# Fable3/CarND-Path-Planning-Project

Hardware: AMD Instinct MI355X
Metric: candidate trajectories/sec (spline+cost, 50-pt horizon) at 1/2/4/8 MI355X (higher is better)
Workload: dtype f64

## Files before the change

carnd-path-planning-project_amd/csrc/pp_api.h:

```cpp
#pragma once

extern "C" {

void pp_params_default(pp_params* p) {
    if (!p) return;
    memset(p, 0, sizeof(*p));
    p->n_points = 50;
    p->n_speeds = 5;
    p->cost_mode = PP_COST_REFERENCE;
    p->emit_paths = 0;
    const double offs[4] = {-4.0, -2.0, 0.0, 2.0};
    for (int i = 0; i < 4; i++) p->speed_offsets[i] = offs[i];
    p->relaxed_acc = 5;
    p->min_relaxed_acc_while_braking = 4;
    p->maximum_acc = 8;
    p->max_speed = 22.2;
    p->car_length = 4.5;
    p->safety_distance = 2;
    p->keep_distance = 10;
    p->keep_distance_leeway = 0.5;
    p->n_draws = 0;
    p->noise_seed = 0x5EED0002ull;
    p->noise_first_scene = 0;
    p->noise_pos_sigma = 0.5;
// ... 151 lines not shown
}

int32_t pp_map_geometry(const pp_map* M, double* out, int32_t n) {
    if (!M || !out || n != M->n) return PP_ERR_ARG;
    memcpy(out, M->ptab.data(), sizeof(double) * (4 + 2 * NL) * (size_t)n);
    return PP_OK;
}

int32_t pp_reserve(pp_map* M, int32_t device, int64_t max_scenes) {
    if (!M || device < 0 || device >= kMaxDev || max_scenes < 0) return PP_ERR_ARG;
    std::lock_guard<std::mutex> lk(M->mu);
    DeviceGuard g(device);
    int rc = dev_init(M, device);
    if (rc) return rc;
    StreamWS& W = M->dev[device].sws[nullptr];
    rc = ensure_ws(W, nullptr, max_scenes);
    return rc ? rc : ensure_rec(W, nullptr, max_scenes);
}

int32_t pp_eval(pp_map* M, const pp_scene_batch* in, const pp_params* prm, pp_result* out,
                int32_t device, void* hip_stream) {
    return eval_impl(M, in, prm, out, device, hip_stream, nullptr);
}

int32_t pp_debug_set(int32_t key, int32_t value) {
    bool ok = false;
    switch (key) {
        case PP_DBG_PREP_GROUP: ok = prep_group_ok(value); break;
        case PP_DBG_PREP_WAVES: ok = value == 0 || value == 3 || value == 4; break;
        case PP_DBG_SHAPE: ok = value >= 0 && value <= PP_SHAPE_STEP; break;
        case PP_DBG_POISON: ok = value == 0 || value == 1; break;
        case PP_DBG_SPLIT: ok = value >= 0 && value <= 2; break;
        case PP_DBG_SORT_CARS: ok = value >= 0 && value <= 2; break;
        default: break;
    }
    if (!ok) return PP_ERR_ARG;
    g_dbg[key].store(value, std::memory_order_relaxed);
    return PP_OK;
}

int32_t pp_debug_get(int32_t key) { return key >= 0 && key < PP_DBG_KEYS ? dbg(key) : PP_ERR_ARG; }

int32_t pp_timing_enable(pp_map* M, int32_t device, int32_t enable) {
    if (!M || device < 0 || device >= kMaxDev) return PP_ERR_ARG;
    std::lock_guard<std::mutex> lk(M->mu);
    DevState& D = M->dev[device];
    D.timing = enable == PP_TIMING_K2 ? 2 : (enable != 0 ? 1 : 0);
    if (D.timing) {
        DeviceGuard g(device);
        const int rc = dev_init(M, device);
        if (rc) return rc;
        while (D.ev.pool.size() + D.ev.rec.size() < 4 * kSplitMax * 256) {
            hipEvent_t e;
            if (hipEventCreate(&e) != hipSuccess) return PP_ERR_HIP;
            D.ev.pool.push_back(e);
        }
    }
    return PP_OK;
}

int32_t pp_timing_read(pp_map* M, int32_t device, double* ms3, int64_t* launches3) {
    if (!M || device < 0 || device >= kMaxDev || !ms3 || !launches3) return PP_ERR_ARG;
    std::lock_guard<std::mutex> lk(M->mu);
    DevState& D = M->dev[device];
    DeviceGuard g(device);
    for (int k = 0; k < 3; k++) { ms3[k] = 0; launches3[k] = 0; }
// ... 117 lines not shown
```

carnd-path-planning-project_amd/csrc/pp_host_map.h:

```cpp
#pragma once

namespace {

constexpr int kMaxDev = 16;
constexpr int kMaxWaypoints = 1 << 24;
constexpr int kPrepD = 12 + 4 * NL;
constexpr int kPrepI = 7;

template <class H, hipError_t (*kRelease)(H)>
class Owned {
    H h_ = nullptr;
public:
    Owned() = default;
    Owned(Owned&& o) noexcept { std::swap(h_, o.h_); }
    Owned& operator=(Owned&& o) noexcept { std::swap(h_, o.h_); return *this; }
    ~Owned() { reset(); }
    H get() const { return h_; }
    explicit operator bool() const { return h_ != nullptr; }
    void reset() { if (h_) (void)kRelease(h_); h_ = nullptr; }
    H* out() { reset(); return &h_; }
};
using Stream = Owned<hipStream_t, hipStreamDestroy>;
using Event = Owned<hipEvent_t, hipEventDestroy>;
struct Pinned : Owned<void*, hipHostFree> {
// ... 12 lines not shown
public:
    DevMem() = default;
    DevMem(DevMem&& o) noexcept { *this = std::move(o); }
    DevMem& operator=(DevMem&& o) noexcept { std::swap(p_, o.p_); std::swap(cap_, o.cap_); return *this; }
    ~DevMem() { reset(); }
    T* get() const { return p_; }
    int64_t cap() const { return cap_; }
    explicit operator bool() const { return p_ != nullptr; }
    void reset() { if (p_) (void)hipFree(p_); p_ = nullptr; cap_ = 0; }
    int grow(hipStream_t st, int64_t cap, size_t bytes) {
        if (cap_ >= cap) return PP_OK;
        if (p_) { (void)hipStreamSynchronize(st); reset(); }
        if (hipMalloc((void**)&p_, bytes) != hipSuccess) { p_ = nullptr; (void)hipGetLastError(); return PP_ERR_NOMEM; }
        cap_ = cap;
        return PP_OK;
    }
    int alloc(size_t n) { return grow(nullptr, (int64_t)n, sizeof(T) * n); }
};
struct EventSet {
    std::vector<hipEvent_t> pool;
    std::vector<hipEvent_t> rec;
    std::vector<int> kind;
    EventSet() = default;
    EventSet(EventSet&& o) noexcept { *this = std::move(o); }
    EventSet& operator=(EventSet&& o) noexcept { pool.swap(o.pool); rec.swap(o.rec); kind.swap(o.kind); return *this; }
    ~EventSet() {
        for (auto* v : {&pool, &rec})
            for (hipEvent_t e : *v) { Event own; *own.out() = e; }
    }
};

constexpr int kSplitMax = 4;
constexpr int kPartMax = 16;
struct StreamWS {
    DevMem<> ws;
    DevMem<> rec;
    DevMem<uint32_t> gbits;
    DevMem<> srt;
    Stream st2[kSplitMax - 1];
    Event fork, join[kSplitMax - 1];
};
struct DevTables {
    DevMem<double> map;
    DevMem<double> lanetab;
    DevMem<uint2> wgrid;
    DevMem<double2> wseg;
    DevMem<double> atab;
};
struct DevRes {
    bool init = false;
    DevTables tab;
    DevMem<double> arctab;
    std::map<void*, StreamWS> sws;
    DevMem<> frame;
    Pinned frame_host;
    Stream frame_stream;
    DevMem<> stage;
    Pinned stage_host;
    EventSet ev;
};
struct DevState : DevRes {
    uint32_t frame_seq = 0;
    std::mutex frame_mu;
    std::mutex stage_mu;
    pptab::CarTable plan_table;
    int timing = 0;
};

}

struct pp_map {
    int n = 0;
    std::vector<double> geom;
    std::vector<double> ptab;
    std::vector<double> lanetab;
    std::vector<double> arctab;
    int fastm = 0;
    std::vector<uint2> wgrid;
    std::vector<double2> wseg;
    std::vector<double> atab;
    WGrid wg;
    DevState dev[kMaxDev];
    std::mutex mu;
};

namespace {

struct DeviceGuard {
    int prev = -1;
    explicit DeviceGuard(int d) { if (hipGetDevice(&prev) != hipSuccess) prev = -1; (void)hipSetDevice(d); }
    ~DeviceGuard() { if (prev >= 0) (void)hipSetDevice(prev); }
};

void fill_arctab(pp_map* M) {
    M->arctab.assign(ppfollow::arc_doubles(M->n), 0.0);
    ppfollow::build_arc(M->lanetab.data() + 2 * NL * (size_t)M->n, M->n, M->arctab.data());
}

void fill_ptab(pp_map* M) {
// ... 284 lines not shown
```

carnd-path-planning-project_amd/csrc/pp_k_cand.h:

```cpp
#pragma once

struct CandRes { double acc_sum, travelled; int ng; uint32_t flags; uint64_t adj0, adj1; };

template <bool kLarge, int kOutMode>
__device__ CandRes run_candidate(const pp_params& P, const Slot& sl, double cx, double cy,
                                 double angle, double ca0, double sa0, SC sc, int room, double* wx,
                                 double* wy, int64_t ws, double* px, int64_t ps, bool out_on = true,
                                 double* rec = nullptr, int dcls = 0, int64_t rs = 0) {
    (void)dcls;
    const bool kOut = kOutMode == 2 || kOutMode == 4;
    const bool kRec = kOutMode == 3 && out_on;
    const int64_t rstride = (int64_t)room * ws;
    CandRes R;
    R.acc_sum = 0; R.travelled = 0; R.ng = 0; R.flags = 0; R.adj0 = 0; R.adj1 = 0;
    const int nk = sl.m(0), ncp = sl.m(1), npk = sl.m(2), mflags = sl.m(3);
    if (mflags & kMetaTrunc) R.flags |= PP_ST_SPLINE_TRUNC;
    if (mflags & kMetaWalkFail) R.flags |= PP_ST_NAN;
    double pos_x = 0, pos_y = 0;
    OutFrame F = {cx, cy, ca0, sa0};
    double opx = cx, opy = cy;
    (void)angle;
    double cur_t = 0.02;
    int ng = 0;
    if (mflags & kMetaFallback) {
// ... 358 lines not shown
    for (int i = K + ng; i < N; i++) {
        if (!PP_CHKP(out.next_x + (int64_t)i * S + s, nx, nnext, 10)) break;
        out.next_x[(int64_t)i * S + s] = 0; out.next_y[(int64_t)i * S + s] = 0;
    }
    out.n_out[s] = K + ng;
    out.winner[s] = c;
}

template <bool kSlow>
__device__ __forceinline__ void cand_status(const PrepV& pv, const pp_result& out, const CandSm& L, int64_t s0,
                                            int nsc, int D, int BPS, int tid) {
    if (tid < nsc && ((L.sSlow[tid] != 0) == kSlow) && PP_CHK(s0 + tid < g_lim.nscen, 15, s0 + tid)) {
        const uint32_t st = (uint32_t)pv.status[(s0 + tid) * D] | L.sFlags[tid];
        if (BPS == 1) out.status[s0 + tid] = st;
        else atomicOr(&out.status[s0 + tid], st);
    }
}

template <bool kSlow>
__device__ __forceinline__ void cand_store_slot(const CandSm& L, int nslot, double* wslot, int64_t s0, int nsc,
                                                int NS, int tid) {
    constexpr int kItems = 5 * kWinKnots + 4;
    for (int idx = tid; idx < nsc * kItems; idx += (int)blockDim.x) {
        const int w = idx / kItems, e = idx - w * kItems;
        if ((L.sSlow[w] != 0) != kSlow) continue;
        const int64_t s = s0 + w;
        const Slot sl = lds_slot(L.sX, nslot, L.sMeta, w * NL + L.sNg[w] / NS);
        double* rec_s = wslot + s * kWinRec;
        if (e < 5 * kWinKnots) rec_s[e] = sl.X[e];
        else ((int*)(rec_s + 5 * kWinKnots))[e - 5 * kWinKnots] = sl.m(e - 5 * kWinKnots);
    }
}

template <bool kSlow, int kMode, int kEmitIn = 0, bool kPreA = false>
__device__ __forceinline__ void cand_group(const MapG& mg, const pp_scene_batch& in, const pp_params& P,
                                           const PrepV& pv, const pp_result& out, int SPB, int BPS,
                                           double* rec, uint64_t* adjm, int64_t g, double* sm,
                                           double* wslot = nullptr) {
    constexpr bool emit_in = kEmitIn == 1 && kMode == 1;
    constexpr bool win_inline = kEmitIn == 2 && kMode == 1;
    const int NS = P.n_speeds, Cv = NL * NS, N = P.n_points;
    const int D = P.n_draws > 1 ? P.n_draws : 1;
    const int C = D * Cv;
    const int nslot = NL * SPB;
    double* sX = sm;
    double* sY = sX + nslot * kKP;
    double* sA = sY + nslot * kKP;
    double* sB = sA + nslot * kKP;
    double* sC = sB + nslot * kKP;
    int* sMeta = (int*)(sC + nslot * kKP);
    uint32_t* sFlags = (uint32_t*)(sMeta + 4 * nslot);
    const MapV m = map_view(mg.buf, mg.n);
    const int64_t S = in.n_scenes;
    const int64_t Sv = S * D;
    int64_t s0;
    int coff;
    int nsc;
    if (BPS == 1) { s0 = g * SPB; coff = 0; }
    else if (BPS < 0) { s0 = g * 256 / C; coff = (int)(g * 256 - s0 * C); }
    else { s0 = g / BPS; coff = (int)(g - s0 * BPS) * 256; }
    if (BPS < 0) {
        const int span = (coff + 255) / C + 1;
        nsc = (int)((S - s0) < span ? (S - s0) : span);
    } else {
        nsc = (int)((S - s0) < SPB ? (S - s0) : SPB);
    }
    const int tid = threadIdx.x;
    uint32_t* sSlow = sFlags + SPB;
    uint64_t* sAdj = (uint64_t*)(((uintptr_t)(sSlow + SPB) + 7) & ~(uintptr_t)7);
    int* sNg = (int*)(sAdj + 2 * SPB);
    double* sCost = (double*)(((uintptr_t)(sNg + SPB) + 7) & ~(uintptr_t)7);
    if (tid < SPB) { sFlags[tid] = 0; sSlow[tid] = 0; }
#ifdef PP_TRACE
    if (!kSlow && tid == 0) {
        PP_TRACE_AT(blockIdx.x, 0);
        if (blockIdx.x < (unsigned)kTraceK1) g_trace[8 * blockIdx.x + 7] = trace_hwid();
    }
#endif
#ifdef PP_CHECK
    if (!kPreA) {
        for (int i = tid; i < 5 * nslot * kKP; i += (int)blockDim.x) sX[i] = __builtin_nan("");
        for (int i = tid; i < 4 * nslot; i += (int)blockDim.x) sMeta[i] = kMetaPoison;
    }
#endif
    __syncthreads();
    bool mine = false;
    for (int t = tid; t < nsc * D; t += (int)blockDim.x) {
        const int q = t / D;
        if (pv.lim_mask[(s0 + q) * D + (t - q * D)] & kLimSlow) { atomicOr(&sSlow[q], 1u); mine = true; }
    }
    if (!__syncthreads_or(mine) && kSlow) return;
    if (!kPreA) {
        int TS = (int)blockDim.x / nslot;
        if (TS > 8) TS = 8;
        const int j = tid / TS, r = tid - j * TS;
        const bool act = j < NL * nsc && ((sSlow[j / NL] != 0) == kSlow);
        const Slot sl = lds_slot(sX, nslot, sMeta, j);
        const int L = j % NL;
        const int64_t s = s0 + j / NL;
        LaneGeom g;
        PP_REGION_A("a1");
        if (act) { g = lane_geom(pv, s * D, Sv, L); team_a1(m, in, g, s, L, sl, r, TS); }
        __syncthreads();
        PP_REGION_A("a2");
        const int js = tid;
        const bool act_s = js < NL * nsc && ((sSlow[js / NL] != 0) == kSlow);
        const Slot sls = lds_slot(sX, nslot, sMeta, js);
        if (act_s) {
            const int64_t vs = (s0 + js / NL) * D;
            LaneGeom gs;
            gs.K = pv.K[vs];
            gs.npk = gs.K > 0 ? gs.K - 1 : 0;
            gs.pos_x = pv.pos_x[vs]; gs.pos_y = pv.pos_y[vs]; gs.ego_d = pv.ego_d[vs];
            team_a2(gs, sls);
        }
        __syncthreads();
        PP_REGION_A("a3");
        if (act) team_a3(sl, r, TS);
        __syncthreads();
        PP_REGION_A("a4");
        if (act_s) team_a4(sls);
        __syncthreads();
        PP_REGION_A("a5");
        if (act) team_a5(sl, r, TS);
// ... 140 lines not shown
            double sr, cr;
            turn_sincos<true>(rt, sr, cr);
            pcr[idx] = cr; psr[idx] = sr;
        }
        __syncthreads();
        if (!kSlow && tid == 0) PP_TRACE_AT(blockIdx.x, 7);
        if (tid < nsc && ((sSlow[tid] != 0) == kSlow)) {
            const int64_t s = s0 + tid;
            emit_scene_pre<kEmitChunk>(in, P, pv, out, rec, s, pv.K[s], sNg[tid], sAdj[2 * tid],
                                          sAdj[2 * tid + 1], pcr + tid * N, psr + tid * N);
        }
    }
}

template <bool kSlow, int kMode>
__global__ __launch_bounds__(256) __attribute__((amdgpu_waves_per_eu(kCandWaves))) void k_cand(MapG mg, pp_scene_batch in, pp_params P, PrepV pv,
                                              pp_result out, int SPB, int BPS, double* rec, uint64_t* adjm,
                                              uint32_t* gbits, int64_t ngroups, const uint32_t* glist,
                                              const uint32_t* gcount, int64_t g0, double* wslot) {
    extern __shared__ __attribute__((aligned(16))) double sm[];
    if (!kSlow) {
        cand_group<false, kMode>(mg, in, P, pv, out, SPB, BPS, rec, adjm, g0 + blockIdx.x, sm, wslot);
        return;
    }
    const uint32_t nl = *gcount;
    for (uint32_t i = blockIdx.x; i < nl; i += gridDim.x) {
        const int64_t g = glist[i];
        if (!PP_CHK(g < ngroups, 21, g)) continue;
        __syncthreads();
        cand_group<true, kMode>(mg, in, P, pv, out, SPB, BPS, rec, adjm, g, sm, wslot);
        if (threadIdx.x == 0) atomicAnd(&gbits[g >> 5], ~(1u << (g & 31)));
    }
}
```

carnd-path-planning-project_amd/csrc/pp_k_spline.h:

```cpp
#pragma once

struct Slot {
    double *X, *Y, *A, *B, *C;
    int* meta;
    int64_t st;
    int64_t mst;
    __device__ __forceinline__ double& x(int i) const { return X[i * st]; }
    __device__ __forceinline__ double& y(int i) const { return Y[i * st]; }
    __device__ __forceinline__ double& a(int i) const { return A[i * st]; }
    __device__ __forceinline__ double& b(int i) const { return B[i * st]; }
    __device__ __forceinline__ double& c(int i) const { return C[i * st]; }
    __device__ __forceinline__ int& m(int k) const { return meta[k * mst]; }
};
__device__ __forceinline__ Slot lds_slot(double* sX, int nslot, int* sMeta, int j) {
    (void)nslot;
    double* b = sX + (int64_t)j * kKP * 5;
    return Slot{b, b + 1, b + 2, b + 3, b + 4, sMeta + 4 * j, 5, 1};
}
constexpr int kCandCostLanes = 256;
struct CandLds {
    int spb;
    static __host__ __device__ constexpr size_t up8(size_t b) { return (b + 7) / 8 * 8; }
    __host__ __device__ constexpr int nslot() const { return NL * spb; }
    __host__ __device__ constexpr int slot_doubles() const { return 5 * kKP * nslot(); }
    __host__ __device__ constexpr size_t meta() const { return sizeof(double) * 5 * kKP * nslot(); }
    __host__ __device__ constexpr size_t flags() const { return meta() + sizeof(int) * 4 * nslot(); }
    __host__ __device__ constexpr size_t slow() const { return flags() + sizeof(uint32_t) * spb; }
    __host__ __device__ constexpr size_t adj() const { return up8(slow() + sizeof(uint32_t) * spb); }
    __host__ __device__ constexpr size_t ng() const { return adj() + sizeof(uint64_t) * 2 * spb; }
    __host__ __device__ constexpr size_t bytes() const { return ng() + sizeof(int) * spb; }
    __host__ __device__ constexpr size_t cost() const { return up8(bytes()); }
    __host__ __device__ constexpr size_t bytes_cost() const { return cost() + sizeof(double) * kCandCostLanes; }
    __host__ __device__ constexpr int doubles() const {
        return (int)(((sizeof(double) * 5 * kKP * (NL * spb) + sizeof(int) * 4 * (NL * spb) + sizeof(uint32_t) * 2 * spb + 7) / 8 * 8 +
                      sizeof(uint64_t) * 2 * spb + sizeof(int) * spb + 7) / 8);
    }
    __host__ __device__ constexpr bool replay_fits(int N) const { return 2 * spb * N <= slot_doubles(); }
};
#if PP_NUM_LANES == 3
static_assert(CandLds{1}.bytes() == 2116 && CandLds{4}.bytes() == 8464 && CandLds{16}.bytes() == 33856, "k_cand's LDS");
static_assert(CandLds{1}.bytes_cost() == 4168 && CandLds{4}.bytes_cost() == 10512 &&
              CandLds{16}.bytes_cost() == 35904, "k_cand's LDS with the cost array");
#elif PP_NUM_LANES == 4
static_assert(CandLds{1}.bytes() == 2812 && CandLds{4}.bytes() == 11248 && CandLds{16}.bytes() == 44992, "k_cand's LDS");
static_assert(CandLds{1}.bytes_cost() == 4864 && CandLds{4}.bytes_cost() == 13296 &&
              CandLds{16}.bytes_cost() == 47040, "k_cand's LDS with the cost array");
#endif
static_assert(8u * CandLds{1}.doubles() >= CandLds{1}.bytes() && 8u * CandLds{4}.doubles() >= CandLds{4}.bytes() &&
              8u * CandLds{16}.doubles() >= CandLds{16}.bytes(), "doubles() covers bytes()");
static_assert(CandLds{1}.doubles() == (CandLds{1}.bytes() + 7) / 8 && CandLds{4}.doubles() == (CandLds{4}.bytes() + 7) / 8 &&
              CandLds{16}.doubles() == (CandLds{16}.bytes() + 7) / 8, "doubles() is bytes() rounded up");
constexpr int kMetaFallback = 1, kMetaTrunc = 2, kMetaWalkFail = 4;

__device__ void setup_lane(const MapV& m, const pp_params& P, const pp_scene_batch& in,
                           const PrepV& pv, int64_t s, int64_t v, int64_t Sv, int L, const Slot& sl) {
    const int64_t S = in.n_scenes;
    const int K = pv.K[v];
    const double pos_x = pv.pos_x[v], pos_y = pv.pos_y[v];
    const double ca = pv.ca_m[v], sa = pv.sa_m[v];
    const double start = pv.ego_speed[v], ego_d = pv.ego_d[v], ego_vd = pv.ego_vd[v];
    const int ref_wp = pv.ref_wp[v];
    const double ratio = pv.ratio[L * Sv + v];
    int flags = 0;
    double min_cpd = start * 1;
    min_cpd = s_max(min_cpd, 5.0);
    const double d_diff = lane_offset(L) - ego_d;
    const double d_acc = 4;
    bool slow = false;
    double lst = 2.0;
    if ((ego_vd < 0) == (d_diff < 0)) {
        const double dmax = ego_vd * ego_vd / d_acc / 2;
// ... 263 lines not shown
```

carnd-path-planning-project_amd/csrc/pp_launch.h:

```cpp
#pragma once

namespace {

size_t prep_bytes(int64_t S) { return ((size_t)S * (kPrepD * 8 + kPrepI * 4) + 255) / 256 * 256; }
size_t rec_bytes(int64_t S) { return (size_t)S * (3 * PP_MAX_POINTS + 2) * 8 + 256; }
static_assert(kWinRec <= 3 * PP_MAX_POINTS + 2, "the stored winner slots share the record's memory");
double* rec_buf(void* rec) { return (double*)rec; }
uint64_t* adj_buf(void* rec, int64_t cap) { return (uint64_t*)((double*)rec + 3 * PP_MAX_POINTS * cap); }

PrepV prep_bind(void* base, int64_t S) {
    PrepV p;
    double* d = (double*)base;
    double** dd[] = {&p.pos_x, &p.pos_y, &p.angle, &p.ca_m, &p.sa_m, &p.ca_p, &p.sa_p,
                     &p.ego_speed, &p.ego_d, &p.ego_vd, &p.in_ts, &p.in_tt};
    int k = 0;
    for (double** q : dd) *q = d + (int64_t)(k++) * S;
    p.ratio = d + (int64_t)(k) * S; k += NL;
    p.l_ts = d + (int64_t)(k) * S; k += NL;
    p.l_tt = d + (int64_t)(k) * S; k += NL;
    p.score = d + (int64_t)(k) * S; k += NL;
    int32_t* ip = (int32_t*)(d + (int64_t)kPrepD * S);
    int32_t** ii[] = {&p.K, &p.ref_wp, &p.T, &p.ego_lane, &p.open_mask, &p.lim_mask, &p.status};
    int m = 0;
    for (int32_t** q : ii) *q = ip + (int64_t)(m++) * S;
    return p;
}

std::atomic<int> g_dbg[PP_DBG_KEYS];
int dbg(int key) { return g_dbg[key].load(std::memory_order_relaxed); }

constexpr int64_t kFusedSmall = 16384;
bool fused_small(int64_t S) {
    const int f = dbg(PP_DBG_SHAPE);
    return f ? f != PP_SHAPE_SPLIT : S <= kFusedSmall;
}
bool step_fused_on() { return dbg(PP_DBG_SHAPE) != PP_SHAPE_CAND_SMALL; }
constexpr int64_t kSplitMin = 131072, kSplitMaxScenes = 1572864;
constexpr int64_t kChunkScenes = 1048576;
bool split_on(int64_t S) {
    const int f = dbg(PP_DBG_SPLIT);
    if (f == 2) return false;
    if (f == 1) return S >= 2048;
    return S >= kSplitMin && S <= kSplitMaxScenes;
}
int split_parts(int64_t S) {
    return S > 393216 ? 3 : 2;
}
int split_chunks(int64_t S) {
    if (S <= kSplitMaxScenes) return 1;
    const int64_t c = (S + kChunkScenes - 1) / kChunkScenes;
    return (int)std::min<int64_t>(c, kPartMax / kSplitMax);
}
int cu_count(int device) {
    static int cus[kMaxDev] = {};
    if (device < 0 || device >= kMaxDev) return 256;
    if (cus[device] == 0) {
        int c = 0;
        if (hipDeviceGetAttribute(&c, hipDeviceAttributeMultiprocessorCount, device) != hipSuccess || c <= 0) c = 256;
        cus[device] = c;
    }
    return cus[device];
}
int step_waves_on(int64_t S, int spb, int device) {
    if ((S + kStepWaveSpb - 1) / kStepWaveSpb <= cu_count(device)) return 1;
    if (spb >= 16 && (S + 15) / 16 <= cu_count(device)) return 2;
    return 0;
}
bool prep_w4(int64_t Sv, int device) {
    const int f = dbg(PP_DBG_PREP_WAVES);
    if (f == 3 || f == 4) return f == 4;
    const int64_t waves = (Sv + 63) / 64, simds = 4LL * cu_count(device);
    const int64_t r3 = (waves + 3 * simds - 1) / (3 * simds), r4 = (waves + 4 * simds - 1) / (4 * simds);
    return 357 * r4 < 150 * r3;
}
constexpr int64_t kEmitSmall = 65536;
bool prep_group_ok(int G) { return G == 0 || G == 1 || G == 2 || G == 4 || G == 8 || G == 16; }
int prep_group(int64_t Sv) {
    const int forced = dbg(PP_DBG_PREP_GROUP);
    if (forced > 0) return forced;
    const int64_t target = 256LL * 4 * 64 * 2;
    int G = 1;
    while (G < 16 && Sv * G * 2 <= target) G *= 2;
    return G;
}

// ... 6 lines not shown
    for (int spb = hi; spb >= 1; spb--) {
        const int t = spb * C;
        const double u = (double)t / (double)(((t + 63) / 64) * 64);
        if (u > bu + 1e-9) { bu = u; best = spb; }
    }
    return best;
}

int ensure_ws(StreamWS& W, hipStream_t st, int64_t Sv) { return W.ws.grow(st, Sv, prep_bytes(Sv)); }

size_t srt_bytes(int64_t S, int rows) { return (size_t)S * ((size_t)rows * (4 * sizeof(double) + sizeof(int)) + 8) + 256; }
int ensure_srt(StreamWS& W, hipStream_t st, int64_t S, int rows, SortedCars& sc) {
    const size_t need = srt_bytes(S, rows);
    const int rc = W.srt.grow(st, (int64_t)need, need);
    if (rc) return rc;
    double* b = (double*)W.srt.get();
    const int64_t n = (int64_t)rows * S;
    sc.x = b; sc.y = b + n; sc.vx = b + 2 * n; sc.vy = b + 3 * n;
    sc.id = (int*)(b + 4 * n);
    sc.order = (uint64_t*)(((uintptr_t)(sc.id + n) + 7) & ~(uintptr_t)7);
    sc.rows = rows;
    return PP_OK;
}

int ensure_rec(StreamWS& W, hipStream_t st, int64_t S) {
    const int64_t cap = (S + 63) & ~(int64_t)63;
    return W.rec.grow(st, cap, rec_bytes(cap));
}

int ensure_gbits(StreamWS& W, hipStream_t st, int64_t ngroups) {
    const int64_t words = (ngroups + 31) / 32;
    if (W.gbits.cap() >= words) return PP_OK;
    const int64_t cap = std::max<int64_t>(words, 1024);
    const size_t bytes = sizeof(uint32_t) * (size_t)(cap + kPartMax + 32 * cap);
    DevMem<uint32_t> g = std::move(W.gbits);
    const int rc = g.grow(st, cap, bytes);
    if (rc) return rc;
    if (hipMemsetAsync(g.get(), 0, bytes, st) != hipSuccess) return PP_ERR_HIP;
    W.gbits = std::move(g);
    return PP_OK;
}

struct CandGeom { int spb, bps, threads; size_t lds; int64_t groups; };
bool cand_flat_ok(int C) { return C >= 13 && C <= 128 && 256 % C != 0; }
CandGeom cand_geom(int C, int64_t S, bool flat = false) {
    CandGeom g;
    if (flat) {
        g.spb = (C + 254) / C + 1;
        g.bps = -1;
        g.threads = 256;
        g.lds = CandLds{g.spb}.bytes();
        g.groups = (S * C + 255) / 256;
        return g;
    }
    g.spb = C <= 256 ? cands_per_block(C) : 1;
    g.bps = C <= 256 ? 1 : (C + 255) / 256;
    g.threads = C <= 256 ? ((g.spb * C + 63) / 64) * 64 : 256;
    g.lds = CandLds{g.spb}.bytes();
    g.groups = g.bps == 1 ? (S + g.spb - 1) / g.spb : S * g.bps;
    return g;
}

int n_draws(const pp_params* p) { return p->n_draws > 1 ? p->n_draws : 1; }

size_t prep_lds_atab(int n) {
    return sizeof(double) * (((kMapArrays * (size_t)n + 1) & ~(size_t)1) + kAtabD * (size_t)n);
}
// ... 11 lines not shown
                   int32_t device) {
    if (!M || !in || !out || !params_ok(prm) || device < 0 || device >= kMaxDev) return PP_ERR_ARG;
    if (in->n_scenes < 0 || in->car_stride < 0 || in->car_stride > PP_MAX_CARS) return PP_ERR_ARG;
    if (in->n_scenes == 0) return PP_OK;
    if (!in->ego_x || !in->ego_y || !in->ego_yaw_deg || !in->ego_speed_mph || !in->prev_x ||
        !in->prev_y || !in->n_prev || !in->prev_target_lane || !in->n_cars ||
        (in->car_stride > 0 && (!in->car_id || !in->car_x || !in->car_y || !in->car_vx || !in->car_vy)))
        return PP_ERR_ARG;
    if (!out->winner || !out->n_out || !out->next_x || !out->next_y || !out->cost || !out->status)
        return PP_ERR_ARG;
    if (prm->emit_paths && !out->paths) return PP_ERR_ARG;
    if (in->tab_valid && (!in->tab_lane || !in->tab_s || !in->tab_d || !in->tab_vs || !in->tab_vd ||
                          !in->tab_vx || !in->tab_vy || prm->n_draws > 1 || in->tab_slots < 0 ||
                          in->tab_slots > PP_MAX_CARS))
        return PP_ERR_ARG;
    return PP_OK;
}

struct EvalPlan {
    int64_t S, Sv;
    int Dn, Cn;
    bool ref_direct;
    CandGeom cg;
    bool fused;
    int step_waves, spb_f;
    int64_t groups_f;
    size_t lds_f;
    bool step_fused;
    int prep_g;
    bool need_rec;
    bool need_wslot;
    bool need_srt;
    bool split;
};
int32_t eval_plan(const pp_map* M, const pp_scene_batch* in, const pp_params* prm, int32_t device, EvalPlan& p) {
    p.S = in->n_scenes;
    p.Dn = n_draws(prm);
    p.Sv = p.S * p.Dn;
    p.ref_direct = prm->cost_mode == PP_COST_REFERENCE && p.Dn == 1;
    p.Cn = p.Dn * NL * prm->n_speeds;
    p.cg = cand_geom(p.Cn, p.S, prm->emit_paths && p.Dn == 1 && cand_flat_ok(p.Cn));
    if (p.cg.groups > 0x7fffffff) return PP_ERR_ARG;
    p.fused = p.ref_direct && !prm->emit_paths && p.cg.bps == 1 && CandLds{p.cg.spb}.replay_fits(prm->n_points) && fused_small(p.S);
    p.step_waves = step_waves_on(p.S, p.cg.spb, device);
    const size_t map_lds = sizeof(double) * (size_t)((kMapArrays * M->n + 1) & ~1);
    auto step_lds = [&](int wv, int spb) {
        return map_lds + (wv != 0 ? sizeof(double) * (size_t)(CandLds{spb}.doubles() + kGeoD * spb) : CandLds{spb}.bytes());
    };
    if (p.step_waves && step_lds(p.step_waves, std::min(p.cg.spb, p.step_waves == 1 ? kStepWaveSpb : 16)) > 65536) p.step_waves = 0;
    p.spb_f = std::min(p.cg.spb, p.step_waves == 1 ? kStepWaveSpb : 256 / 16);
    p.groups_f = (p.S + p.spb_f - 1) / p.spb_f;
    p.lds_f = step_lds(p.step_waves, p.spb_f);
    p.step_fused = p.fused && M->n <= kLdsMapMax && p.lds_f <= 65536 && step_fused_on();
    p.prep_g = prep_group(p.Sv);
    p.need_rec = p.ref_direct && !prm->emit_paths;
    p.need_wslot = !p.ref_direct && !prm->emit_paths && p.cg.bps == 1 && p.Dn == 1;
    p.need_srt = dbg(PP_DBG_SORT_CARS) == 1 && !in->tab_valid && p.Dn < kSortDmax && in->car_stride >= 2 &&
                 in->car_stride <= 16 && p.prep_g == 1;
    p.split = p.ref_direct && !prm->emit_paths && !p.fused && p.cg.bps == 1 && p.Dn == 1 && p.prep_g == 1 &&
              split_on(p.S);
    return PP_OK;
}

struct EvalArgs {
    hipStream_t st;
    int32_t device;
    MapG mg;
    pp_scene_batch B;
    pp_params P;
    pp_result R;
    PrepV pv;
    GroupBits gb = {};
    double* rec = nullptr;
    uint64_t* adjm = nullptr;
    double* wslot = nullptr;
    size_t cand_lds;
    SortedCars srt = {};
};

int32_t eval_bind(const pp_map* M, const DevState& DS, StreamWS& W, const pp_scene_batch* in,
                  const pp_params* prm, const pp_result* out, int32_t device, void* hip_stream,
                  const EvalPlan& p, EvalArgs& A) {
    A.st = (hipStream_t)hip_stream;
    A.device = device;
    int rc = ensure_ws(W, A.st, p.Sv);
    if (rc) return rc;
    rc = ensure_gbits(W, A.st, p.cg.groups);
    if (rc) return rc;
    if (p.need_rec) {
        rc = ensure_rec(W, A.st, p.S);
        if (rc) return rc;
        A.rec = rec_buf(W.rec.get());
        A.adjm = adj_buf(W.rec.get(), W.rec.cap());
    }
    if (p.need_srt) {
        rc = ensure_srt(W, A.st, p.S, in->car_stride, A.srt);
        if (rc) return rc;
    }
    A.cand_lds = p.cg.lds;
    if (p.need_wslot) {
        rc = ensure_rec(W, A.st, p.S);
        if (rc) return rc;
        A.wslot = rec_buf(W.rec.get());
        A.cand_lds = CandLds{p.cg.spb}.bytes_cost();
    }
    A.pv = prep_bind(W.ws.get(), W.ws.cap());
    A.mg.buf = DS.tab.map.get();
    A.mg.n = M->n;
    A.mg.fastm = M->fastm;
    A.mg.wg = M->wg;
    A.mg.wg.cells = DS.tab.wgrid.get();
    A.mg.wseg = DS.tab.wseg.get();
    A.mg.atab = DS.tab.atab.get();
    A.mg.atab_lds = DS.tab.atab && prep_lds_atab(M->n) <= 65536;
    A.P = *prm;
    A.B = *in;
    A.R = *out;
    if (!A.P.emit_paths) { A.R.paths = nullptr; A.R.path_len = nullptr; }
    A.gb.bits = W.gbits.get(); A.gb.SPB = p.cg.spb; A.gb.BPS = p.cg.bps; A.gb.C = p.Cn;
    A.gb.count = W.gbits.get() + W.gbits.cap();
    A.gb.list = A.gb.count + kPartMax;
    return PP_OK;
}

int32_t poison_fill(const StreamWS& W, hipStream_t st, const EvalPlan& p, const pp_params* prm,
                    const pp_result* out) {
    auto fill = [&](void* q, size_t bytes) { return !q || !bytes || hipMemsetAsync(q, 0xFF, bytes, st) == hipSuccess; };
    const int64_t S = p.S, Cn = p.Cn, N = prm->n_points;
    const int64_t words = (p.cg.groups + 31) / 32;
    std::vector<uint32_t> hb((size_t)words);
    if (hipMemcpyAsync(hb.data(), W.gbits.get(), sizeof(uint32_t) * words, hipMemcpyDeviceToHost, st) != hipSuccess ||
        hipStreamSynchronize(st) != hipSuccess)
        return PP_ERR_HIP;
    for (uint32_t w : hb)
        if (w) return PP_ERR_STATE;
    const bool ok = fill(W.ws.get(), prep_bytes(W.ws.cap())) &&
                    fill(W.rec.get(), W.rec ? rec_bytes(W.rec.cap()) : 0) &&
                    fill(W.srt.get(), (size_t)W.srt.cap()) &&
                    fill(W.gbits.get() + W.gbits.cap() + kPartMax, sizeof(uint32_t) * 32 * (size_t)W.gbits.cap()) &&
                    fill(out->winner, 4 * S) && fill(out->n_out, 4 * S) && fill(out->status, 4 * S) &&
                    fill(out->next_x, 8 * N * S) && fill(out->next_y, 8 * N * S) &&
                    fill(out->cost, 8 * Cn * S) && fill(out->info, sizeof(pp_scene_info) * S) &&
                    fill(out->draw_mean_cost, p.Dn > 1 ? 8 * NL * prm->n_speeds * S : 0) &&
                    fill(prm->emit_paths ? out->paths : nullptr, 16 * N * Cn * S) &&
                    fill(prm->emit_paths ? out->path_len : nullptr, 4 * Cn * S);
    return ok ? PP_OK : PP_ERR_HIP;
}

#ifdef PP_CHECK
int32_t check_limits(const StreamWS& W, const EvalPlan& p, const EvalArgs& A) {
    ChkLim L = {};
    const long long Cn = p.Cn;
    L.paths = A.R.paths; L.npaths = A.R.paths ? (long long)p.S * A.P.n_points * Cn * 2 : 0;
    L.nx = A.R.next_x; L.ny = A.R.next_y; L.nnext = (long long)p.S * A.P.n_points;
    L.rec = A.rec; L.nrec = A.rec ? 3LL * PP_MAX_POINTS * W.rec.cap() : 0;
    L.adjm = (const unsigned long long*)A.adjm; L.nadj = A.adjm ? 2LL * W.rec.cap() : 0;
    L.cost = A.R.cost; L.ncost = (long long)p.S * Cn; L.nscen = p.S;
    if (hipDeviceSynchronize() != hipSuccess ||
        hipMemcpyToSymbol(HIP_SYMBOL(g_lim), &L, sizeof L) != hipSuccess) return PP_ERR_HIP;
    return PP_OK;
}
#endif

struct EvalEvents { DevState* DS; size_t base; bool timing, tall, tk2; };
hipEvent_t ev_at(const EvalEvents& E, int i) {
    DevState& DS = *E.DS;
    hipEvent_t& e = DS.ev.rec[E.base + i];
    if (!e) {
        if (DS.ev.pool.empty() && hipEventCreate(&e) != hipSuccess) return nullptr;
        if (!e) { e = DS.ev.pool.back(); DS.ev.pool.pop_back(); }
    }
    return e;
// ... 86 lines not shown
        for (int h = 0; h < NS; h++) {
            const int t = c * NS + h;
            hipStream_t sh = h == 0 ? st : W.st2[h - 1].get();
            const int64_t g0 = G * t / NT, g1 = G * (t + 1) / NT;
            const int64_t v0 = std::min<int64_t>(S, g0 * cg.spb), v1 = std::min<int64_t>(S, g1 * cg.spb);
            if (v1 <= v0) continue;
            GroupBits gbh = A.gb;
            gbh.count = A.gb.count + t;
            gbh.list = A.gb.list + g0;
            const int eh = 4 * launched++;
            if (E.tall) (void)hipEventRecord(ev_at(E, eh), sh);
            const unsigned pb = (unsigned)((v1 - v0 + 255) / 256);
            if (A.srt.rows)
                hipLaunchKernelGGL(k_sort_cars, dim3(pb), dim3(256), 0, sh, A.B, A.srt, v0, v1);
            launch_prep(A, sh, v0, v1, gbh, A.srt, L);
            if (E.tk2) (void)hipEventRecord(ev_at(E, eh + 1), sh);
            const unsigned nsl = (unsigned)std::min<int64_t>(g1 - g0, 2048);
            launch_cand<1>(A, sh, cg, (unsigned)(g1 - g0), nsl, gbh.list, gbh.count, g0);
            if (E.tk2) (void)hipEventRecord(ev_at(E, eh + 2), sh);
            hipLaunchKernelGGL(k_emit<kEmitRows>, dim3(pb), dim3(256), 0, sh, A.B, A.P, A.pv, A.R,
                               A.rec, A.adjm, v0, v1);
            if (E.tall) (void)hipEventRecord(ev_at(E, eh + 3), sh);
        }
        for (int k = 0; k < NS - 1; k++)
            if (hipEventRecord(W.join[k].get(), W.st2[k].get()) != hipSuccess || hipStreamWaitEvent(st, W.join[k].get(), 0) != hipSuccess)
                return PP_ERR_HIP;
    }
    if (E.timing) E.DS->ev.kind.back() |= (launched << 8) | (NC > 1 ? NS << 16 : 0);
    g_dbg[PP_DBG_LAST_PARTS].store(launched, std::memory_order_relaxed);
    if (hipGetLastError() != hipSuccess) return PP_ERR_HIP;
    return PP_OK;
}

int32_t launch_plain(const EvalArgs& A, const EvalPlan& p, const EvalEvents& E) {
    hipStream_t st = A.st;
    const CandGeom& cg = p.cg;
    const int64_t S = p.S, Sv = p.Sv;
    {
        const int G = p.prep_g;
        const int64_t blocks = (Sv * G + 255) / 256;
        if (E.tall) (void)hipEventRecord(ev_at(E, 0), st);
        const PrepLds L = prep_lds(A.mg);
        switch (G) {
            case 2: launch_prep_grp(k_prep_g2<true>, k_prep_g2<false>, A, blocks, L); break;
            case 4: launch_prep_grp(k_prep_g4<true>, k_prep_g4<false>, A, blocks, L); break;
            case 8: launch_prep_grp(k_prep_g8<true>, k_prep_g8<false>, A, blocks, L); break;
            case 16: launch_prep_grp(k_prep_g16<true>, k_prep_g16<false>, A, blocks, L); break;
            default:
                if (A.srt.rows)
                    hipLaunchKernelGGL(k_sort_cars, dim3((unsigned)((S + 255) / 256)), dim3(256), 0, st, A.B, A.srt, (int64_t)0, S);
                launch_prep(A, st, 0, Sv, A.gb, A.srt, L);
                break;
        }
    }
    {
        const unsigned nb = (unsigned)cg.groups;
        const unsigned nslow = (unsigned)std::min<int64_t>(cg.groups, 2048);
        if (E.tk2) (void)hipEventRecord(ev_at(E, 1), st);
        if (A.P.emit_paths) launch_cand<2>(A, st, cg, nb, nslow, A.gb.list, A.gb.count, 0);
        else if (p.ref_direct && p.fused) {
            hipLaunchKernelGGL(k_cand_small, dim3(nb), dim3(cg.threads), cg.lds, st, A.mg, A.B, A.P, A.pv, A.R,
                               cg.spb, A.rec, A.adjm, A.gb.bits);
        }
        else if (p.ref_direct) launch_cand<1>(A, st, cg, nb, nslow, A.gb.list, A.gb.count, 0);
        else launch_cand<0>(A, st, cg, nb, nslow, A.gb.list, A.gb.count, 0);
    }
    if (E.tk2) (void)hipEventRecord(ev_at(E, 2), st);
    if (p.ref_direct && !A.P.emit_paths && !p.fused) {
        if (S <= kEmitSmall) {
            const int64_t blocks = (S + 63) / 64;
            hipLaunchKernelGGL(k_emit<16>, dim3((unsigned)blocks), dim3(64), 0, st, A.B, A.P, A.pv, A.R, A.rec, A.adjm, (int64_t)0, S);
        } else {
            const int64_t blocks = (S + 255) / 256;
            hipLaunchKernelGGL(k_emit<kEmitRows>, dim3((unsigned)blocks), dim3(256), 0, st, A.B, A.P, A.pv, A.R, A.rec, A.adjm, (int64_t)0, S);
        }
    }
    if (!p.ref_direct) {
        const int64_t blocks = (S + kWinBlock - 1) / kWinBlock;
        if (A.wslot) {
            const unsigned b256 = (unsigned)((S + 255) / 256);
            hipLaunchKernelGGL((k_winner_st<false>), dim3(b256), dim3(256), 0, st, A.B, A.P, A.pv, A.R, (const double*)A.wslot);
            hipLaunchKernelGGL((k_winner_st<true>), dim3(b256), dim3(256), 0, st, A.B, A.P, A.pv, A.R, (const double*)A.wslot);
        } else {
            hipLaunchKernelGGL((k_winner<false>), dim3((unsigned)blocks), dim3(kWinBlock), 0, st, A.mg, A.B, A.P, A.pv, A.R);
            hipLaunchKernelGGL((k_winner<true>), dim3((unsigned)blocks), dim3(kWinBlock), 0, st, A.mg, A.B, A.P, A.pv, A.R);
        }
    }
    if (E.tall) (void)hipEventRecord(ev_at(E, 3), st);
    if (hipGetLastError() != hipSuccess) return PP_ERR_HIP;
    return PP_OK;
}

int32_t eval_impl(pp_map* M, const pp_scene_batch* in, const pp_params* prm, pp_result* out,
                  int32_t device, void* hip_stream, const FrameIO* fio) {
    int32_t rc = eval_check(M, in, prm, out, device);
    if (rc || in->n_scenes == 0) return rc;
    DeviceGuard g(device);
    EvalPlan p;
    rc = eval_plan(M, in, prm, device, p);
    if (rc) return rc;
    if (fio && (!p.step_fused || p.groups_f != 1)) return PP_ERR_STATE;
    std::lock_guard<std::mutex> lk(M->mu);
    rc = dev_init(M, device);
    if (rc) return rc;
    DevState& DS = M->dev[device];
    StreamWS& W = DS.sws[hip_stream];
    EvalArgs A;
    rc = eval_bind(M, DS, W, in, prm, out, device, hip_stream, p, A);
    if (rc) return rc;
    if (dbg(PP_DBG_POISON)) {
        rc = poison_fill(W, A.st, p, prm, out);
        if (rc) return rc;
    }
    EvalEvents E = {&DS, DS.ev.rec.size(), DS.timing != 0, DS.timing == 1, DS.timing != 0};
    if (E.timing) {
        DS.ev.rec.resize(E.base + 4 * kPartMax, nullptr);
        DS.ev.kind.push_back((!(p.ref_direct && prm->emit_paths) && !p.fused ? 1 : 0) | (E.tall ? 0 : 16));
    }
#ifdef PP_CHECK
    rc = check_limits(W, p, A);
    if (rc) return rc;
#endif
    if (p.step_fused) return launch_step(A, p, E, fio);
    if (hipMemsetAsync(A.gb.count, 0, kPartMax * sizeof(uint32_t), A.st) != hipSuccess) return PP_ERR_HIP;
    g_dbg[PP_DBG_LAST_PARTS].store(1, std::memory_order_relaxed);
    return p.split ? launch_split(A, p, E, W) : launch_plain(A, p, E);
}

}
```

carnd-path-planning-project_amd/ppamd/__init__.py:

```python
from __future__ import annotations

import ctypes as C
import os

import numpy as np

_HERE = os.path.dirname(os.path.abspath(__file__))
LIB_PATH = os.environ.get("PPAMD_LIB") or os.path.join(_HERE, "libppamd.so")


def lib_sha256(path=None):
    import hashlib
    h = hashlib.sha256()
    with open(path or LIB_PATH, "rb") as f:
        for b in iter(lambda: f.read(1 << 20), b""):
            h.update(b)
    return h.hexdigest()

def _open():
    if not os.path.exists(LIB_PATH):
        raise ImportError(f"ppamd: HIP library not built: {LIB_PATH} (run __graft_entry__.build())")
    try:
        import torch
    except ImportError:
# ... 720 lines not shown


def plan_frame(m: Map, ego_x, ego_y, ego_yaw_deg, ego_speed_mph, prev_x, prev_y, cars,
               target_lane=1, device=0):
    px = np.ascontiguousarray(prev_x, np.float64)
    py = np.ascontiguousarray(prev_y, np.float64)
    rows = [tuple(r)[:5] for r in cars]
    ids = np.array([int(r[0]) for r in rows], np.int32)
    cx = np.array([r[1] for r in rows], np.float64)
    cy = np.array([r[2] for r in rows], np.float64)
    cvx = np.array([r[3] for r in rows], np.float64)
    cvy = np.array([r[4] for r in rows], np.float64)
    tl = C.c_int32(target_lane)
    nx = np.zeros(50, np.float64)
    ny = np.zeros(50, np.float64)
    n_out = C.c_int32(0)
    _check(lib.pp_plan_frame(m.handle, device, ego_x, ego_y, ego_yaw_deg, ego_speed_mph,
                             px.ctypes.data_as(_dp), py.ctypes.data_as(_dp), len(px),
                             ids.ctypes.data_as(_ip), cx.ctypes.data_as(_dp),
                             cy.ctypes.data_as(_dp), cvx.ctypes.data_as(_dp),
                             cvy.ctypes.data_as(_dp), len(rows), C.byref(tl),
                             nx.ctypes.data_as(_dp), ny.ctypes.data_as(_dp), C.byref(n_out)),
           "pp_plan_frame")
    n = n_out.value
    return nx[:n].copy(), ny[:n].copy(), tl.value


DATA_DIR = os.path.join(os.path.dirname(_HERE), "data")


TIMING_ALL, TIMING_K2 = 1, 2

DBG_PREP_GROUP, DBG_PREP_WAVES, DBG_SHAPE, DBG_POISON, DBG_SPLIT, DBG_LAST_PARTS, DBG_SORT_CARS = 0, 1, 2, 3, 4, 5, 6
SPLIT_AUTO, SPLIT_ON, SPLIT_OFF = 0, 1, 2
SHAPE_AUTO, SHAPE_SPLIT, SHAPE_CAND_SMALL, SHAPE_STEP = 0, 1, 2, 3


def debug_set(key, value):
    _check(lib.pp_debug_set(key, value), "pp_debug_set")


def debug_get(key):
    return lib.pp_debug_get(key)


class debug:

    def __init__(self, key, value):
        self.key, self.value = key, value

    def __enter__(self):
        self.prev = debug_get(self.key)
        debug_set(self.key, self.value)
        return self

    def __exit__(self, *exc):
        debug_set(self.key, self.prev)
        return False


def set_prep_group(lanes):
    debug_set(DBG_PREP_GROUP, lanes)


def highway_map():
    z = np.load(os.path.join(DATA_DIR, "highway_map.npz"))
    return z["x"].copy(), z["y"].copy()
# ... 173 lines not shown
```

include/pp.h:

```cpp
#ifndef PP_H
#define PP_H

#include <stdint.h>

#ifdef __cplusplus
extern "C" {
#endif

#ifndef PP_NUM_LANES
#define PP_NUM_LANES   3
#endif
#define PP_PREV_KEEP   10
#if PP_NUM_LANES <= 3
#define PP_MAX_CARS    256
#else
#define PP_MAX_CARS    64
#endif
#define PP_NOISE_CAR_STRIDE 256
#define PP_MAX_SPEEDS  8
#define PP_MAX_POINTS  128
#define PP_MAX_KNOTS   16
#define PP_MAX_DRAWS   1024

#define PP_OK              0
// ... 286 lines not shown
int32_t pp_telemetry_parse(const char* buf, const int64_t* offsets, int64_t n_msgs, pp_scene_batch* out,
                           int32_t* msg_status, int32_t n_threads);
int32_t pp_control_format(const double* next_x, const double* next_y, const int32_t* n_out, int64_t n_scenes,
                          int64_t stride, char* out, int64_t out_cap, int64_t* offsets, int32_t n_threads);

int32_t pp_telemetry_parse_device(const char* d_buf, const int64_t* d_offsets, int64_t n_msgs, pp_scene_batch* d_out,
                                  int32_t* d_status, int32_t device, void* hip_stream);
int32_t pp_control_format_device(const double* d_next_x, const double* d_next_y, const int32_t* d_n_out,
                                 int64_t n_scenes, int64_t stride, char* d_slots, int64_t slot_bytes,
                                 int32_t* d_len, int32_t device, void* hip_stream);

typedef struct pp_server_opts {
    const char* host;
    int32_t port;
    int32_t max_clients;
    int32_t n_speeds;
    int32_t threads;
    int32_t device;
    int32_t _pad;
    int64_t max_frames;
} pp_server_opts;

int32_t pp_serve(pp_map* m, const pp_server_opts* opts, volatile int32_t* stop, int32_t* bound_port,
                 int64_t* stats);
int32_t pp_ws_accept_key(const char* key, char* out, int32_t cap);

#define PP_DBG_PREP_GROUP  0
#define PP_DBG_PREP_WAVES  1
#define PP_DBG_SHAPE       2
#define PP_DBG_POISON      3
#define PP_DBG_SPLIT       4
#define PP_DBG_LAST_PARTS  5
#define PP_DBG_SORT_CARS   6
#define PP_DBG_KEYS        7
#define PP_SHAPE_SPLIT      1
#define PP_SHAPE_CAND_SMALL 2
#define PP_SHAPE_STEP       3
int32_t pp_debug_set(int32_t key, int32_t value);
int32_t pp_debug_get(int32_t key);

#define PP_TIMING_ALL 1
#define PP_TIMING_K2  2
int32_t pp_timing_enable(pp_map* m, int32_t device, int32_t enable);
int32_t pp_timing_read(pp_map* m, int32_t device, double* ms3, int64_t* launches3);

double  pp_mc_gauss(uint64_t seed, int64_t scene, int32_t draw, int32_t car, int32_t q);

int32_t pp_libm_eval(int32_t kind, const double* a, const double* b, double* out, int64_t n,
                     int32_t device, void* hip_stream);

enum {
    PP_MATH_SINCOS = 0, PP_MATH_SINCOS_NOLARGE, PP_MATH_ATAN2_PP, PP_MATH_ATAN2_FAST, PP_MATH_ATAN2_UNIT,
    PP_MATH_ASIN_SMALL, PP_MATH_RCP_NR, PP_MATH_DIV_RCP, PP_MATH_DIV_RCP_NC, PP_MATH_DIV_RCP_AUTO,
    PP_MATH_DIV_RCP_NC_AUTO, PP_MATH_DIV50, PP_MATH_DIV50_NC, PP_MATH_SQRT_RD, PP_MATH_DIV_RCP_N,
    PP_MATH_DIV_RCP_D, PP_MATH_FMOD_2PI, PP_MATH_FMOD_2PI_SMALL, PP_MATH_TURN_SINCOS,
    PP_MATH_TURN_SINCOS_NOLARGE, PP_MATH_SINCOS_SMALL, PP_MATH_TURN_ANGLE, PP_MATH_TURN_ANGLE_NOLARGE,
    PP_MATH_TURN_ANGLE_FAST, PP_MATH_SC_SPEED, PP_MATH_SC_SPEED_R, PP_MATH_SC_SPEED_R_NC,
    PP_MATH_SC_OVERRIDE, PP_MATH_SC_OVERRIDE_R, PP_MATH_SC_OVERRIDE_R_NC, PP_MATH_SPEED_IN_RANGE,
    PP_MATH_KINDS
};
int32_t pp_math_eval(int32_t kind, const double* a, const double* b, const double* c, const double* d,
                     double* out0, double* out1, double* out2, int64_t n, int32_t device, void* hip_stream);

const char* pp_version(void);

#ifdef __cplusplus
}
// ... 3 lines not shown
```

Before: 3.209 billion.

## Add persistent work-stealing k_cand kernel for large reference-mode batches

Adds a persistent variant of the candidate kernel sized to occupancy times CU count. Each block pulls further scene groups from a global atomic counter instead of one block being launched per group. It runs only the fast path and a separate slow-path kernel follows. It is enabled automatically above the split-threshold scene count, aiming to cut block launch/tail overhead and improve load balance. It adds atomic contention and an extra barrier per group, and changes how the counter area of the gbits buffer is laid out.

```diff
diff --git a/carnd-path-planning-project_amd/csrc/pp_api.h b/carnd-path-planning-project_amd/csrc/pp_api.h
--- a/carnd-path-planning-project_amd/csrc/pp_api.h
+++ b/carnd-path-planning-project_amd/csrc/pp_api.h
@@ -207,6 +207,7 @@
         case PP_DBG_POISON: ok = value == 0 || value == 1; break;
         case PP_DBG_SPLIT: ok = value >= 0 && value <= 2; break;
         case PP_DBG_SORT_CARS: ok = value >= 0 && value <= 2; break;
+        case PP_DBG_PERSIST: ok = value >= 0 && value <= 2; break;
         default: break;
     }
     if (!ok) return PP_ERR_ARG;
diff --git a/carnd-path-planning-project_amd/csrc/pp_host_map.h b/carnd-path-planning-project_amd/csrc/pp_host_map.h
--- a/carnd-path-planning-project_amd/csrc/pp_host_map.h
+++ b/carnd-path-planning-project_amd/csrc/pp_host_map.h
@@ -68,6 +68,7 @@
 
 constexpr int kSplitMax = 4;
 constexpr int kPartMax = 16;
+constexpr int kPersistCtr = 2;
 struct StreamWS {
     DevMem<> ws;
     DevMem<> rec;
@@ -101,6 +102,8 @@
     std::mutex stage_mu;
     pptab::CarTable plan_table;
     int timing = 0;
+    int persist_blocks = 0, persist_threads = 0;
+    size_t persist_lds = 0;
 };
 
 }
diff --git a/carnd-path-planning-project_amd/csrc/pp_k_cand.h b/carnd-path-planning-project_amd/csrc/pp_k_cand.h
--- a/carnd-path-planning-project_amd/csrc/pp_k_cand.h
+++ b/carnd-path-planning-project_amd/csrc/pp_k_cand.h
@@ -414,7 +414,7 @@
     }
 }
 
-template <bool kSlow, int kMode, int kEmitIn = 0, bool kPreA = false>
+template <bool kSlow, int kMode, int kEmitIn = 0, bool kPreA = false, bool kLoop = false>
 __device__ __forceinline__ void cand_group(const MapG& mg, const pp_scene_batch& in, const pp_params& P,
                                            const PrepV& pv, const pp_result& out, int SPB, int BPS,
                                            double* rec, uint64_t* adjm, int64_t g, double* sm,
@@ -447,7 +447,8 @@
     } else {
         nsc = (int)((S - s0) < SPB ? (S - s0) : SPB);
     }
-    const int tid = threadIdx.x;
+    int tid = threadIdx.x;
+    if (kLoop) asm volatile("" : "+v"(tid));
     uint32_t* sSlow = sFlags + SPB;
     uint64_t* sAdj = (uint64_t*)(((uintptr_t)(sSlow + SPB) + 7) & ~(uintptr_t)7);
     int* sNg = (int*)(sAdj + 2 * SPB);
@@ -471,7 +472,8 @@
         const int q = t / D;
         if (pv.lim_mask[(s0 + q) * D + (t - q * D)] & kLimSlow) { atomicOr(&sSlow[q], 1u); mine = true; }
     }
-    if (!__syncthreads_or(mine) && kSlow) return;
+    if (kLoop && !kSlow) __syncthreads();
+    else if (!__syncthreads_or(mine) && kSlow) return;
     if (!kPreA) {
         int TS = (int)blockDim.x / nslot;
         if (TS > 8) TS = 8;
@@ -678,3 +680,28 @@
         if (threadIdx.x == 0) atomicAnd(&gbits[g >> 5], ~(1u << (g & 31)));
     }
 }
+
+struct Persist {};
+struct PersistArgs {
+    MapG mg; pp_scene_batch in; pp_params P; PrepV pv; pp_result out;
+    int SPB; double* rec; uint64_t* adjm; int64_t ngroups; uint32_t* next;
+};
+template <class kTag, int kMode>
+__global__ __launch_bounds__(256) __attribute__((amdgpu_waves_per_eu(kCandWaves))) void k_cand(PersistArgs a0) {
+    static_assert(kMode == 1, "the persistent K2 is reference mode's");
+    typedef const __attribute__((address_space(4))) PersistArgs* KArg;
+    extern __shared__ __attribute__((aligned(16))) double sm[];
+    int64_t g = blockIdx.x;
+    if (g >= a0.ngroups) return;
+    for (;;) {
+        KArg ka = (KArg)__builtin_amdgcn_kernarg_segment_ptr();
+        asm volatile("" : "+s"(ka));
+        const PersistArgs& a = *(const PersistArgs*)ka;
+        cand_group<false, kMode, 0, false, true>(a.mg, a.in, a.P, a.pv, a.out, a.SPB, 1, a.rec, a.adjm, g, sm, nullptr);
+        uint32_t* sNext = (uint32_t*)(sm + CandLds{a.SPB}.doubles());
+        if (threadIdx.x == 0) *sNext = atomicAdd(a.next, 1u);
+        __syncthreads();
+        g = (int64_t)gridDim.x + *sNext;
+        if (g >= a.ngroups) return;
+    }
+}
diff --git a/carnd-path-planning-project_amd/csrc/pp_k_spline.h b/carnd-path-planning-project_amd/csrc/pp_k_spline.h
--- a/carnd-path-planning-project_amd/csrc/pp_k_spline.h
+++ b/carnd-path-planning-project_amd/csrc/pp_k_spline.h
@@ -36,7 +36,9 @@
                       sizeof(uint64_t) * 2 * spb + sizeof(int) * spb + 7) / 8);
     }
     __host__ __device__ constexpr bool replay_fits(int N) const { return 2 * spb * N <= slot_doubles(); }
+    __host__ __device__ constexpr size_t bytes_persist() const { return sizeof(double) * (size_t)doubles() + 8; }
 };
+static_assert(PP_NUM_LANES != 3 || 4 * CandLds{17}.bytes_persist() <= 160 * 1024, "four persistent k_cand blocks per CU");
 #if PP_NUM_LANES == 3
 static_assert(CandLds{1}.bytes() == 2116 && CandLds{4}.bytes() == 8464 && CandLds{16}.bytes() == 33856, "k_cand's LDS");
 static_assert(CandLds{1}.bytes_cost() == 4168 && CandLds{4}.bytes_cost() == 10512 &&
diff --git a/carnd-path-planning-project_amd/csrc/pp_launch.h b/carnd-path-planning-project_amd/csrc/pp_launch.h
--- a/carnd-path-planning-project_amd/csrc/pp_launch.h
+++ b/carnd-path-planning-project_amd/csrc/pp_launch.h
@@ -51,6 +51,11 @@
     const int64_t c = (S + kChunkScenes - 1) / kChunkScenes;
     return (int)std::min<int64_t>(c, kPartMax / kSplitMax);
 }
+constexpr int64_t kPersistMinScenes = kSplitMaxScenes + 1;
+bool persist_on(int64_t S) {
+    const int f = dbg(PP_DBG_PERSIST);
+    return f == 1 || (f == 0 && S >= kPersistMinScenes);
+}
 int cu_count(int device) {
     static int cus[kMaxDev] = {};
     if (device < 0 || device >= kMaxDev) return 256;
@@ -123,7 +128,7 @@
     const int64_t words = (ngroups + 31) / 32;
     if (W.gbits.cap() >= words) return PP_OK;
     const int64_t cap = std::max<int64_t>(words, 1024);
-    const size_t bytes = sizeof(uint32_t) * (size_t)(cap + kPartMax + 32 * cap);
+    const size_t bytes = sizeof(uint32_t) * (size_t)(cap + kPartMax + kPersistCtr + 32 * cap);
     DevMem<uint32_t> g = std::move(W.gbits);
     const int rc = g.grow(st, cap, bytes);
     if (rc) return rc;
@@ -201,6 +206,7 @@
     bool need_wslot;
     bool need_srt;
     bool split;
+    bool persist;
 };
 int32_t eval_plan(const pp_map* M, const pp_scene_batch* in, const pp_params* prm, int32_t device, EvalPlan& p) {
     p.S = in->n_scenes;
@@ -228,6 +234,8 @@
                  in->car_stride <= 16 && p.prep_g == 1;
     p.split = p.ref_direct && !prm->emit_paths && !p.fused && p.cg.bps == 1 && p.Dn == 1 && p.prep_g == 1 &&
               split_on(p.S);
+    p.persist = p.ref_direct && !prm->emit_paths && !p.fused && !p.split && p.cg.bps == 1 && p.Dn == 1 &&
+                persist_on(p.S);
     return PP_OK;
 }
 
@@ -245,6 +253,8 @@
     double* wslot = nullptr;
     size_t cand_lds;
     SortedCars srt = {};
+    uint32_t* next = nullptr;
+    unsigned persist = 0;
 };
 
 int32_t eval_bind(const pp_map* M, const DevState& DS, StreamWS& W, const pp_scene_batch* in,
@@ -288,7 +298,8 @@
     if (!A.P.emit_paths) { A.R.paths = nullptr; A.R.path_len = nullptr; }
     A.gb.bits = W.gbits.get(); A.gb.SPB = p.cg.spb; A.gb.BPS = p.cg.bps; A.gb.C = p.Cn;
     A.gb.count = W.gbits.get() + W.gbits.cap();
-    A.gb.list = A.gb.count + kPartMax;
+    A.next = A.gb.count + kPartMax;
+    A.gb.list = A.next + kPersistCtr;
     return PP_OK;
 }
 
@@ -306,7 +317,7 @@
     const bool ok = fill(W.ws.get(), prep_bytes(W.ws.cap())) &&
                     fill(W.rec.get(), W.rec ? rec_bytes(W.rec.cap()) : 0) &&
                     fill(W.srt.get(), (size_t)W.srt.cap()) &&
-                    fill(W.gbits.get() + W.gbits.cap() + kPartMax, sizeof(uint32_t) * 32 * (size_t)W.gbits.cap()) &&
+                    fill(W.gbits.get() + W.gbits.cap() + kPartMax + kPersistCtr, sizeof(uint32_t) * 32 * (size_t)W.gbits.cap()) &&
                     fill(out->winner, 4 * S) && fill(out->n_out, 4 * S) && fill(out->status, 4 * S) &&
                     fill(out->next_x, 8 * N * S) && fill(out->next_y, 8 * N * S) &&
                     fill(out->cost, 8 * Cn * S) && fill(out->info, sizeof(pp_scene_info) * S) &&
@@ -459,6 +470,22 @@
     return PP_OK;
 }
 
+unsigned persist_blocks(DevState& DS, const CandGeom& cg, int device) {
+    const size_t lds = CandLds{cg.spb}.bytes_persist();
+    if (DS.persist_blocks == 0 || DS.persist_threads != cg.threads || DS.persist_lds != lds) {
+        int nb = 0;
+        if (hipOccupancyMaxActiveBlocksPerMultiprocessor(&nb, k_cand<Persist, 1>, cg.threads, lds) != hipSuccess || nb < 1) {
+            (void)hipGetLastError();
+            nb = 1;
+        }
+        nb = std::min(nb, std::max(1, 4 * kCandWaves * 64 / cg.threads));
+        DS.persist_blocks = nb * cu_count(device);
+        DS.persist_threads = cg.threads;
+        DS.persist_lds = lds;
+    }
+    return (unsigned)DS.persist_blocks;
+}
+
 int32_t launch_plain(const EvalArgs& A, const EvalPlan& p, const EvalEvents& E) {
     hipStream_t st = A.st;
     const CandGeom& cg = p.cg;
@@ -489,6 +516,13 @@
             hipLaunchKernelGGL(k_cand_small, dim3(nb), dim3(cg.threads), cg.lds, st, A.mg, A.B, A.P, A.pv, A.R,
                                cg.spb, A.rec, A.adjm, A.gb.bits);
         }
+        else if (p.ref_direct && A.persist) {
+            const PersistArgs pa = {A.mg, A.B, A.P, A.pv, A.R, cg.spb, A.rec, A.adjm, cg.groups, A.next};
+            hipLaunchKernelGGL((k_cand<Persist, 1>), dim3(std::min(A.persist, nb)), dim3(cg.threads),
+                               CandLds{cg.spb}.bytes_persist(), st, pa);
+            hipLaunchKernelGGL((k_cand<true, 1>), dim3(nslow), dim3(cg.threads), A.cand_lds, st, A.mg, A.B, A.P, A.pv, A.R,
+                               cg.spb, cg.bps, A.rec, A.adjm, A.gb.bits, cg.groups, A.gb.list, A.gb.count, (int64_t)0, A.wslot);
+        }
         else if (p.ref_direct) launch_cand<1>(A, st, cg, nb, nslow, A.gb.list, A.gb.count, 0);
         else launch_cand<0>(A, st, cg, nb, nslow, A.gb.list, A.gb.count, 0);
     }
@@ -548,8 +582,10 @@
     rc = check_limits(W, p, A);
     if (rc) return rc;
 #endif
+    A.persist = p.persist && !p.step_fused ? persist_blocks(DS, p.cg, device) : 0;
+    g_dbg[PP_DBG_LAST_PERSIST].store((int)A.persist, std::memory_order_relaxed);
     if (p.step_fused) return launch_step(A, p, E, fio);
-    if (hipMemsetAsync(A.gb.count, 0, kPartMax * sizeof(uint32_t), A.st) != hipSuccess) return PP_ERR_HIP;
+    if (hipMemsetAsync(A.gb.count, 0, (kPartMax + kPersistCtr) * sizeof(uint32_t), A.st) != hipSuccess) return PP_ERR_HIP;
     g_dbg[PP_DBG_LAST_PARTS].store(1, std::memory_order_relaxed);
     return p.split ? launch_split(A, p, E, W) : launch_plain(A, p, E);
 }
diff --git a/carnd-path-planning-project_amd/ppamd/__init__.py b/carnd-path-planning-project_amd/ppamd/__init__.py
--- a/carnd-path-planning-project_amd/ppamd/__init__.py
+++ b/carnd-path-planning-project_amd/ppamd/__init__.py
@@ -776,7 +776,9 @@
 TIMING_ALL, TIMING_K2 = 1, 2
 
 DBG_PREP_GROUP, DBG_PREP_WAVES, DBG_SHAPE, DBG_POISON, DBG_SPLIT, DBG_LAST_PARTS, DBG_SORT_CARS = 0, 1, 2, 3, 4, 5, 6
+DBG_PERSIST, DBG_LAST_PERSIST = 7, 8
 SPLIT_AUTO, SPLIT_ON, SPLIT_OFF = 0, 1, 2
+PERSIST_AUTO, PERSIST_ON, PERSIST_OFF = 0, 1, 2
 SHAPE_AUTO, SHAPE_SPLIT, SHAPE_CAND_SMALL, SHAPE_STEP = 0, 1, 2, 3
 
 
diff --git a/include/pp.h b/include/pp.h
--- a/include/pp.h
+++ b/include/pp.h
@@ -342,7 +342,9 @@
 #define PP_DBG_SPLIT       4
 #define PP_DBG_LAST_PARTS  5
 #define PP_DBG_SORT_CARS   6
-#define PP_DBG_KEYS        7
+#define PP_DBG_PERSIST     7
+#define PP_DBG_LAST_PERSIST 8
+#define PP_DBG_KEYS        9
 #define PP_SHAPE_SPLIT      1
 #define PP_SHAPE_CAND_SMALL 2
 #define PP_SHAPE_STEP       3
```

Result: faster. 3.306 billion (median of 6 runs) (+3.0%).
